# mokemokechicken/reversi-alpha-zero

Measured on AMD Instinct MI355X. Metric: MCTS simulations/sec (self-play, NN included), higher is better.
Workload: dtype f64 tree statistics + f32 net (f16x3 split-operand MFMA trunk)

## Files before the change

### reversi-alpha-zero_amd/csrc/raz_leaf_cache.hip

```cpp
#include <hip/hip_runtime.h>
#include <string.h>
#include "raz_engine.h"
#include "raz_internal.h"

namespace {

constexpr uint32_t kProbes = 8;
enum : uint32_t { ROLE_NONE = 0, ROLE_PLAIN = 1, ROLE_OWN = 2, ROLE_FOLLOW = 3, ROLE_WAIT = 4 };

__device__ __forceinline__ unsigned long long leaf_tag(unsigned long long a, unsigned long long b) {
    unsigned long long x = a * 0x9E3779B97F4A7C15ULL ^ (b + 0xD6E8FEB86659FD93ULL) * 0xC2B2AE3D27D4EB4FULL;
    x ^= x >> 32; x *= 0xFF51AFD7ED558CCDULL; x ^= x >> 29; x *= 0xC4CEB9FE1A85EC53ULL; x ^= x >> 32;
    return x | 1ULL;
}

__global__ __launch_bounds__(256) void k_leaf_claim(raz_leaf_cache_dev C, const unsigned long long* __restrict__ own,
                                                    const unsigned long long* __restrict__ enemy, const uint8_t* __restrict__ active,
                                                    uint32_t p0, uint32_t pn, uint32_t part, uint32_t step) {
    const uint32_t j = blockIdx.x * 256 + threadIdx.x;
    if (j == 0) C.n_compact[part] = 0;
    if (j >= pn) return;
    const uint32_t r = p0 + j;
    if (!active[r]) {
        C.role[r] = ROLE_NONE;
        return;
    }
    const unsigned long long o = own[r], e = enemy[r], tag = leaf_tag(o, e);
    if ((uint32_t)__popcll(o | e) > C.max_discs) {
        C.role[r] = ROLE_PLAIN;
        return;
    }
    const uint32_t h = (uint32_t)(tag >> 24) & C.mask;
    uint32_t role = ROLE_PLAIN;
    for (uint32_t k = 0; k < kProbes; ++k) {
        const uint32_t i = (h + k) & C.mask;
        unsigned long long t = __hip_atomic_load(&C.tags[i], __ATOMIC_RELAXED, __HIP_MEMORY_SCOPE_AGENT);
        if (t == 0) {
            t = atomicCAS(&C.tags[i], 0ULL, tag);
            if (t == 0) {
                C.keys[2 * (size_t)i] = o;
                C.keys[2 * (size_t)i + 1] = e;
                C.stamp[i] = step;
                C.owner[i] = r;
                role = (i << 3) | ROLE_OWN;
                break;
            }
        }
        if (t == tag) {
            role = (i << 3) | ROLE_FOLLOW;
            break;
        }
    }
    if (role == ROLE_PLAIN) atomicAdd(&C.counters[3], 1ULL);
    C.role[r] = role;
}

__global__ __launch_bounds__(256) void k_leaf_resolve(raz_leaf_cache_dev C, const unsigned long long* __restrict__ own,
                                                      const unsigned long long* __restrict__ enemy, uint8_t* __restrict__ active,
                                                      float* __restrict__ policy, float* __restrict__ value, uint32_t p0, uint32_t pn,
                                                      uint32_t part, uint32_t step) {
    const uint32_t j = blockIdx.x * 4 + (threadIdx.x >> 6), lane = threadIdx.x & 63;
    if (j >= pn) return;
    const uint32_t r = p0 + j;
    uint32_t role = __builtin_amdgcn_readfirstlane(C.role[r]);
    const uint32_t kind = role & 7u, i = role >> 3;
    if (kind == ROLE_NONE) return;
    if (kind == ROLE_FOLLOW) {
        const bool same = C.keys[2 * (size_t)i] == own[r] && C.keys[2 * (size_t)i + 1] == enemy[r];
        const uint32_t ow = C.owner[i];
        if (same && __hip_atomic_load(&C.ready[i], __ATOMIC_ACQUIRE, __HIP_MEMORY_SCOPE_AGENT)) {
            policy[(size_t)r * 64 + lane] = C.pv[(size_t)i * 72 + lane];
            if (lane == 0) {
                value[r] = C.pv[(size_t)i * 72 + 64];
                active[r] = 0;
                C.role[r] = ROLE_NONE;
                atomicAdd(&C.counters[0], 1ULL);
            }
            return;
        }
        if (same && C.stamp[i] == step && ow >= p0 && ow < p0 + pn && ow != r) {
            if (lane == 0) {
                active[r] = 0;
                C.role[r] = (i << 3) | ROLE_WAIT;
                atomicAdd(&C.counters[1], 1ULL);
            }
            return;
        }
        role = ROLE_PLAIN;
        if (lane == 0) C.role[r] = ROLE_PLAIN;
    }
    if (lane == 0) {
        const uint32_t ci = atomicAdd(&C.n_compact[part], 1u);
        C.list[p0 + ci] = j;
        atomicAdd(&C.counters[2], 1ULL);
    }
}

__global__ __launch_bounds__(256) void k_leaf_fill(raz_leaf_cache_dev C, float* __restrict__ policy, float* __restrict__ value,
                                                   uint32_t p0, uint32_t pn, uint32_t step) {
    const uint32_t j = blockIdx.x * 4 + (threadIdx.x >> 6), lane = threadIdx.x & 63;
    if (j >= pn) return;
    const uint32_t r = p0 + j, role = C.role[r], kind = role & 7u, i = role >> 3;
    if (kind == ROLE_OWN) {
        if (C.stamp[i] != step || C.owner[i] != r) return;
        C.pv[(size_t)i * 72 + lane] = policy[(size_t)r * 64 + lane];
        if (lane == 0) {
            C.pv[(size_t)i * 72 + 64] = value[r];
            __hip_atomic_store(&C.ready[i], 1u, __ATOMIC_RELEASE, __HIP_MEMORY_SCOPE_AGENT);
        }
    } else if (kind == ROLE_WAIT) {
        const uint32_t ow = C.owner[i];
        policy[(size_t)r * 64 + lane] = policy[(size_t)ow * 64 + lane];
        if (lane == 0) value[r] = value[ow];
    }
}

}

size_t raz_leaf_cache_layout(uint32_t log2_entries, size_t rows, unsigned char* base, raz_leaf_cache_dev* out) {
    const size_t E = (size_t)1 << log2_entries;
    size_t off = 0;
    auto take = [&](size_t bytes) -> unsigned char* {
        unsigned char* p = base ? base + off : nullptr;
        off = (off + bytes + 255) / 256 * 256;
        return p;
    };
    raz_leaf_cache_dev c;
    memset(&c, 0, sizeof c);
    c.tags = (unsigned long long*)take(E * 8);
    c.keys = (unsigned long long*)take(E * 16);
    c.stamp = (uint32_t*)take(E * 4);
    c.owner = (uint32_t*)take(E * 4);
    c.ready = (uint32_t*)take(E * 4);
    c.pv = (float*)take(E * 72 * 4);
    c.counters = (unsigned long long*)take(8 * 8);
    c.n_compact = (uint32_t*)take(16 * 4);
    c.list = (uint32_t*)take(rows * 4);
    c.role = (uint32_t*)take(rows * 4);
    c.mask = (uint32_t)(E - 1);
    c.entries = (uint32_t)E;
    if (out) *out = c;
    return off;
}

int raz_leaf_cache_clear(const raz_leaf_cache_dev& c, size_t rows, hipStream_t s) {
    const size_t E = (size_t)c.entries;
    RAZ_HIP_TRY(hipMemsetAsync(c.tags, 0, E * 8, s), "leaf cache: clear tags");
    RAZ_HIP_TRY(hipMemsetAsync(c.ready, 0, E * 4, s), "leaf cache: clear ready flags");
    RAZ_HIP_TRY(hipMemsetAsync(c.stamp, 0, E * 4, s), "leaf cache: clear stamps");
    RAZ_HIP_TRY(hipMemsetAsync(c.counters, 0, 64, s), "leaf cache: clear counters");
    RAZ_HIP_TRY(hipMemsetAsync(c.n_compact, 0, 64, s), "leaf cache: clear counts");
    RAZ_HIP_TRY(hipMemsetAsync(c.role, 0, rows * 4, s), "leaf cache: clear roles");
    return RAZ_OK;
}

int raz_leaf_cache_before(const raz_leaf_cache_dev& c, const raz_engine_dev& d, uint32_t p0, uint32_t pn, uint32_t part, uint32_t step,
                          hipStream_t s) {
    hipLaunchKernelGGL(k_leaf_claim, dim3((pn + 255) / 256), dim3(256), 0, s, c, d.nn_own, d.nn_enemy, d.nn_active, p0, pn, part, step);
    hipLaunchKernelGGL(k_leaf_resolve, dim3((pn + 3) / 4), dim3(256), 0, s, c, d.nn_own, d.nn_enemy, d.nn_active, d.nn_policy, d.nn_value,
                       p0, pn, part, step);
    return raz_check_launch("raz_engine_step: leaf cache lookup");
}

int raz_leaf_cache_after(const raz_leaf_cache_dev& c, const raz_engine_dev& d, uint32_t p0, uint32_t pn, uint32_t step, hipStream_t s) {
    hipLaunchKernelGGL(k_leaf_fill, dim3((pn + 3) / 4), dim3(256), 0, s, c, d.nn_policy, d.nn_value, p0, pn, step);
    return raz_check_launch("raz_engine_step: leaf cache fill");
}

extern "C" int raz_leaf_cache_probe(int phase, void* d_cache, size_t bytes, uint32_t log2_entries, uint32_t max_discs, size_t rows,
                                    const uint64_t* d_own, const uint64_t* d_enemy, uint8_t* d_active, float* d_policy, float* d_value,
                                    uint32_t p0, uint32_t pn, uint32_t part, uint32_t step, raz_stream_t stream) {
    if (phase < 0 || phase > 2) return raz_fail(RAZ_EINVAL, "raz_leaf_cache_probe: unknown phase");
    if (log2_entries < 10 || log2_entries > 28) return raz_fail(RAZ_EINVAL, "raz_leaf_cache_probe: log2_entries must be 10..28");
    if (!d_cache || ((uintptr_t)d_cache & 255)) return raz_fail(RAZ_EINVAL, "raz_leaf_cache_probe: cache buffer NULL or not 256-byte aligned");
    if (bytes < raz_leaf_cache_layout(log2_entries, rows, nullptr, nullptr)) return raz_fail(RAZ_EINVAL, "raz_leaf_cache_probe: buffer too small (raz_leaf_cache_bytes)");
    if (!d_own || !d_enemy || !d_active || !d_policy || !d_value) return raz_fail(RAZ_EINVAL, "raz_leaf_cache_probe: NULL row buffer");
    if (((uintptr_t)d_own & 7) || ((uintptr_t)d_enemy & 7) || ((uintptr_t)d_policy & 3) || ((uintptr_t)d_value & 3))
        return raz_fail(RAZ_EINVAL, "raz_leaf_cache_probe: misaligned row buffer");
    if ((size_t)p0 + pn > rows) return raz_fail(RAZ_EINVAL, "raz_leaf_cache_probe: slice beyond the rows");
    if (part >= 16) return raz_fail(RAZ_EINVAL, "raz_leaf_cache_probe: part must be below 16");
    if (phase != 0 && pn == 0) return raz_fail(RAZ_EINVAL, "raz_leaf_cache_probe: empty slice");
    raz_leaf_cache_dev c;
    raz_leaf_cache_layout(log2_entries, rows, (unsigned char*)d_cache, &c);
    c.max_discs = max_discs ? max_discs : 64u;
    if (phase == 0) return raz_leaf_cache_clear(c, rows, (hipStream_t)stream);
    raz_engine_dev d;
    memset(&d, 0, sizeof d);
    d.nn_own = (unsigned long long*)d_own;
    d.nn_enemy = (unsigned long long*)d_enemy;
    d.nn_active = d_active;
    d.nn_policy = d_policy;
    d.nn_value = d_value;
    if (phase == 1) return raz_leaf_cache_before(c, d, p0, pn, part, step, (hipStream_t)stream);
    return raz_leaf_cache_after(c, d, p0, pn, step, (hipStream_t)stream);
}
```

### reversi-alpha-zero_amd/csrc/raz_net_f16x3.hip

```cpp
#include <hip/hip_runtime.h>
#include <math.h>
#include <stdlib.h>
#include <string.h>
#include <vector>
#include "raz_bitboard.h"
#include "raz_detmath.h"
#include "raz_internal.h"
#include "raz_net_layout.h"

namespace {

typedef _Float16 h8 __attribute__((ext_vector_type(8)));
typedef _Float16 h4 __attribute__((ext_vector_type(4)));
typedef float f32x4 __attribute__((ext_vector_type(4)));
typedef float f32x16 __attribute__((ext_vector_type(16)));

constexpr int OCT = 128;
constexpr int NWAVE = 8;
constexpr int W_STAGE = 3 * 2 * 2 * OCT * 16;
constexpr int ACT_POS = 4 * 64 * 16;
constexpr int ACT_IMG = NWAVE * ACT_POS + 1280;
constexpr int LDS_W = 0;
constexpr int LDS_ACT = 2 * W_STAGE;
constexpr int LDS_BYTES = LDS_ACT + 2 * ACT_IMG;
constexpr int Z_OFF = NWAVE * ACT_POS;

#ifdef RAZ_F16X3_STAMPS
#define RAZ_STAMP_PARAM , unsigned long long* __restrict__ stamps
#define RAZ_STAMP_ARG , (unsigned long long*)nullptr
#define RAZ_STAMP_BEGIN                                                                                           \
    unsigned long long st_t[8];                                                                                   \
    st_t[0] = __builtin_amdgcn_s_memtime();                                                                       \
    st_t[7] = __builtin_amdgcn_s_memrealtime();                                                                   \
    st_t[6] = (unsigned long long)__builtin_amdgcn_s_getreg((4 << 0) | (0 << 6) | (31 << 11)) | ((unsigned long long)__builtin_amdgcn_s_getreg((20 << 0) | (0 << 6) | (31 << 11)) << 32); \
    st_t[5] = 0;                                                                                                  \
    st_t[1] = st_t[2] = st_t[3] = st_t[4] = 0;                                                                    \
    unsigned long long st_b = 0
#define RAZ_STAMP_BARRIER_IN st_b = __builtin_amdgcn_s_memtime()
#define RAZ_STAMP_BARRIER_OUT(st_)                                    \
    do {                                                              \
        const unsigned long long t_ = __builtin_amdgcn_s_memtime();   \
        st_t[5] += t_ - st_b;                                         \
        if ((st_) == 0) st_t[1] = t_;                                 \
    } while (0)
#define RAZ_STAMP_AT(i_) st_t[i_] = __builtin_amdgcn_s_memtime()
#define RAZ_STAMP_END                                                                                    \
    do {                                                                                                 \
        st_t[3] = __builtin_amdgcn_s_memtime();                                                          \
        __builtin_amdgcn_s_waitcnt(0x0070);                                                \
        st_t[4] = __builtin_amdgcn_s_memtime();                                                          \
        if (lane == 0 && stamps)                                                                         \
            for (int i_ = 0; i_ < 8; ++i_) stamps[((size_t)blockIdx.x * NWAVE + wv) * 8 + i_] = st_t[i_]; \
    } while (0)
#else
#define RAZ_STAMP_PARAM
#define RAZ_STAMP_ARG
#define RAZ_STAMP_BEGIN
#define RAZ_STAMP_BARRIER_IN
#define RAZ_STAMP_BARRIER_OUT(st_)
#define RAZ_STAMP_AT(i_)
#define RAZ_STAMP_END
#endif

#define GLDS16(gptr, lptr)                                                                                      \
    __builtin_amdgcn_global_load_lds((const __attribute__((address_space(1))) void*)(gptr),                     \
                                     (__attribute__((address_space(3))) void*)(lptr), 16, 0, 0)

template <bool SPLIT>
__global__ __launch_bounds__(512, 2) void k_conv3x3_f16x3(const unsigned char* __restrict__ Wl, const float* __restrict__ bias,
                                                          const float* __restrict__ inv_scale_ptr, const unsigned char* in, unsigned char* out,
                                                          const unsigned char* skip, const uint8_t* __restrict__ active, int n, int F,
                                                          unsigned* __restrict__ flag, const uint32_t* __restrict__ n_ptr RAZ_STAMP_PARAM) {
    extern __shared__ __attribute__((aligned(16))) unsigned char lds[];
    const int tid = threadIdx.x, lane = tid & 63, wv = tid >> 6;
    RAZ_STAMP_BEGIN;
    if (n_ptr) n = (int)*n_ptr < n ? (int)*n_ptr : n;
    const int noct = F / OCT, nchunks = F / 16;
    const int b = blockIdx.x;
    const int ot = (b >> 3) % noct;
    const int pg = (b / (8 * noct)) * 8 + (b & 7);
    const int p0 = pg * NWAVE, pos = p0 + wv;
    if (p0 >= n) return;
    const bool live = pos < n && (!active || active[pos]);
    const size_t pos_bytes = (size_t)F * 256;
    const unsigned char* in_pos = in + (size_t)(pos < n ? pos : n - 1) * pos_bytes;
    if (tid < 160) {
        const int im = tid / 80, k = tid % 80;
        ((f32x4*)(lds + LDS_ACT + im * ACT_IMG + Z_OFF))[k] = (f32x4){0.f, 0.f, 0.f, 0.f};
    }
    const int kg = lane >> 5;
    uint32_t boff[2][9];
#pragma unroll
    for (int nt = 0; nt < 2; ++nt) {
        const int sq = nt * 32 + (lane & 31), y = sq >> 3, x = sq & 7;
#pragma unroll
        for (int t = 0; t < 9; ++t) {
            const int yy = y + t / 3 - 1, xx = x + t % 3 - 1;
            const bool ok = yy >= 0 && yy < 8 && xx >= 0 && xx < 8;
            const int s2 = sq + (t / 3 - 1) * 8 + (t % 3 - 1);
            boff[nt][t] = ok ? (uint32_t)(wv * ACT_POS + kg * 2048 + s2 * 16) : (uint32_t)(Z_OFF + (s2 & 15) * 16);
        }
    }
    const uint32_t aoff = (uint32_t)(kg * 4096 + (lane & 31) * 16);
    f32x16 acc[4][2];
#pragma unroll
    for (int m = 0; m < 4; ++m)
#pragma unroll
        for (int nt = 0; nt < 2; ++nt)
#pragma unroll
            for (int r = 0; r < 16; ++r) acc[m][nt][r] = 0.f;
    const unsigned char* wsrc = Wl + (size_t)ot * nchunks * 3 * W_STAGE + lane * 16;
    const unsigned char* asrc = in_pos + lane * 16;
    auto issue = [&](int c, int tg) {
        const int st = c * 3 + tg;
        const unsigned char* src = wsrc + (size_t)st * W_STAGE;
        unsigned char* dst = lds + LDS_W + (st & 1) * W_STAGE;
        if constexpr (SPLIT) {
#pragma unroll
            for (int i = 0; i < 3; ++i) GLDS16(src + (wv * 3 + i) * 1024, dst + (wv * 3 + i) * 1024);
        } else {
            const int p0w = (wv >> 1) * 4 + (wv & 1);
            GLDS16(src + p0w * 1024, dst + p0w * 1024);
            if (wv < 4) GLDS16(src + (p0w + 16) * 1024, dst + (p0w + 16) * 1024);
        }
        if (tg == 0) {
            const unsigned char* a = asrc + (size_t)c * ACT_POS;
            unsigned char* ad = lds + LDS_ACT + (c & 1) * ACT_IMG + wv * ACT_POS;
#pragma unroll
            for (int pl = 0; pl < 4; pl += SPLIT ? 1 : 2) GLDS16(a + pl * 1024, ad + pl * 1024);
        }
    };
    issue(0, 0);
    for (int c = 0; c < nchunks; ++c) {
        const uint32_t abase = (uint32_t)(LDS_ACT + (c & 1) * ACT_IMG);
#pragma unroll
        for (int tg = 0; tg < 3; ++tg) {
            const int st = c * 3 + tg;
            RAZ_STAMP_BARRIER_IN;
            __syncthreads();
            RAZ_STAMP_BARRIER_OUT(st);
            if (tg < 2) issue(c, tg + 1);
            else if (c + 1 < nchunks) issue(c + 1, 0);
            const uint32_t wbase = (uint32_t)(LDS_W + (st & 1) * W_STAGE) + aoff;
#pragma unroll
            for (int tt = 0; tt < 3; ++tt) {
                const int t = tg * 3 + tt;
                if constexpr (SPLIT) {
                    h8 bh[2], bl[2];
#pragma unroll
                    for (int nt = 0; nt < 2; ++nt) {
                        bh[nt] = *(const h8*)(lds + abase + boff[nt][t]);
                        bl[nt] = *(const h8*)(lds + abase + boff[nt][t] + 1024);
                    }
#pragma unroll
                    for (int m = 0; m < 4; ++m) {
                        const h8 ah = *(const h8*)(lds + wbase + tt * 8192 + m * 512);
                        const h8 al = *(const h8*)(lds + wbase + tt * 8192 + m * 512 + 2048);
#pragma unroll
                        for (int nt = 0; nt < 2; ++nt) {
                            acc[m][nt] = __builtin_amdgcn_mfma_f32_32x32x16_f16(al, bh[nt], acc[m][nt], 0, 0, 0);
                            acc[m][nt] = __builtin_amdgcn_mfma_f32_32x32x16_f16(ah, bl[nt], acc[m][nt], 0, 0, 0);
                            acc[m][nt] = __builtin_amdgcn_mfma_f32_32x32x16_f16(ah, bh[nt], acc[m][nt], 0, 0, 0);
                        }
                    }
                } else {
                    h8 bh[2];
#pragma unroll
                    for (int nt = 0; nt < 2; ++nt) bh[nt] = *(const h8*)(lds + abase + boff[nt][t]);
#pragma unroll
                    for (int m = 0; m < 4; ++m) {
                        const h8 ah = *(const h8*)(lds + wbase + tt * 8192 + m * 512);
#pragma unroll
                        for (int nt = 0; nt < 2; ++nt) acc[m][nt] = __builtin_amdgcn_mfma_f32_32x32x16_f16(ah, bh[nt], acc[m][nt], 0, 0, 0);
                    }
                }
            }
        }
    }
    RAZ_STAMP_AT(2);
    if (!live) return;
    const float inv_scale = *inv_scale_ptr;
    unsigned char* out_pos = out + (size_t)pos * pos_bytes;
    const unsigned char* skip_pos = skip ? skip + (size_t)pos * pos_bytes : nullptr;
    bool over = false;
#pragma unroll
    for (int m = 0; m < 4; ++m)
#pragma unroll
        for (int q = 0; q < 4; ++q) {
            const int oc8 = ot * OCT + m * 32 + q * 8;
            const f32x4 bv = *(const f32x4*)(bias + oc8 + 4 * kg);
            const size_t unit = (size_t)(oc8 >> 4) * ACT_POS + (size_t)((oc8 >> 3) & 1) * 2048;
#pragma unroll
            for (int nt = 0; nt < 2; ++nt) {
                const size_t o = unit + (size_t)(nt * 32 + (lane & 31)) * 16 + kg * 8;
                float v[4];
#pragma unroll
                for (int j = 0; j < 4; ++j) v[j] = acc[m][nt][q * 4 + j] * inv_scale + bv[j];
                if (skip_pos) {
                    if constexpr (SPLIT) {
                        const h4 sh = *(const h4*)(skip_pos + o), sl = *(const h4*)(skip_pos + o + 1024);
#pragma unroll
                        for (int j = 0; j < 4; ++j) v[j] = v[j] + ((float)sh[j] + (float)sl[j]);
                    } else {
                        const h4 sh = *(const h4*)(skip_pos + o);
#pragma unroll
                        for (int j = 0; j < 4; ++j) v[j] = v[j] + (float)sh[j];
                    }
                }
                h4 hi, lo;
#pragma unroll
                for (int j = 0; j < 4; ++j) {
                    const float r = v[j] > 0.0f ? v[j] : 0.0f;
                    over |= !(r < 60000.0f);
                    hi[j] = (_Float16)r;
                    lo[j] = (_Float16)(r - (float)hi[j]);
                }
                *(h4*)(out_pos + o) = hi;
                if constexpr (SPLIT) *(h4*)(out_pos + o + 1024) = lo;
            }
        }
    if (over) flag[(size_t)pos * RAZ_NET_ROWFLAG_WORDS] = 1u;
    RAZ_STAMP_END;
}

template <bool SPLIT>
__global__ __launch_bounds__(256) void k_conv0_split(const float* __restrict__ W0, const raz_bb* __restrict__ own,
                                                     const raz_bb* __restrict__ enemy, const uint8_t* __restrict__ active,
                                                     unsigned char* out, int n, int F, unsigned* __restrict__ flag,
                                                     const uint32_t* __restrict__ list, const uint32_t* __restrict__ n_ptr) {
    const int pos = blockIdx.x, lane = threadIdx.x & 63;
    const int wv = __builtin_amdgcn_readfirstlane(threadIdx.x >> 6);
    if (threadIdx.x == 0) {
        flag[(size_t)pos * RAZ_NET_ROWFLAG_WORDS] = 0u;
        if (pos == 0) flag[1] = 0u;
    }
    __syncthreads();
    if (n_ptr) n = (int)*n_ptr < n ? (int)*n_ptr : n;
    if (pos >= n || (!list && active && !active[pos])) return;
    bool over = false;
    const size_t src = list ? list[pos] : (size_t)pos;
    const raz_bb bo = own[src], be = enemy[src];
    const int y = lane >> 3, x = lane & 7;
    float x0[9], x1[9];
#pragma unroll
    for (int t = 0; t < 9; ++t) {
        const int yy = y + t / 3 - 1, xx = x + t % 3 - 1;
        const bool ok = (yy >= 0) && (yy < 8) && (xx >= 0) && (xx < 8);
        const int s = (yy * 8 + xx) & 63;
        x0[t] = ok ? (float)((bo >> s) & 1) : 0.0f;
        x1[t] = ok ? (float)((be >> s) & 1) : 0.0f;
    }
    const float* bias = W0 + (size_t)F * 18;
    unsigned char* op = out + (size_t)pos * F * 256;
    for (int ocb = wv; ocb < F / 16; ocb += 4) {
        float acc[16];
#pragma unroll
        for (int o = 0; o < 16; ++o) acc[o] = bias[ocb * 16 + o];
#pragma unroll
        for (int t = 0; t < 9; ++t) {
            const float* wt = W0 + ((size_t)ocb * 9 + t) * 32;
#pragma unroll
            for (int o = 0; o < 16; ++o) acc[o] = fmaf(x0[t], wt[o], acc[o]);
#pragma unroll
            for (int o = 0; o < 16; ++o) acc[o] = fmaf(x1[t], wt[16 + o], acc[o]);
        }
#pragma unroll
        for (int g = 0; g < 2; ++g) {
            h8 hi, lo;
#pragma unroll
            for (int j = 0; j < 8; ++j) {
                const float r = acc[g * 8 + j] > 0.0f ? acc[g * 8 + j] : 0.0f;
                over |= !(r < 60000.0f);
                hi[j] = (_Float16)r;
                lo[j] = (_Float16)(r - (float)hi[j]);
            }
            *(h8*)(op + (size_t)ocb * ACT_POS + (g * 2 + 0) * 1024 + lane * 16) = hi;
            if constexpr (SPLIT) *(h8*)(op + (size_t)ocb * ACT_POS + (g * 2 + 1) * 1024 + lane * 16) = lo;
        }
    }
    if (over) flag[(size_t)pos * RAZ_NET_ROWFLAG_WORDS] = 1u;
}

template <bool SPLIT>
__global__ __launch_bounds__(64) void k_heads_split(const float* __restrict__ H, const unsigned char* trunk,
                                                    const uint8_t* __restrict__ active, float* __restrict__ policy,
                                                    float* __restrict__ value, int n, int F, int V,
                                                    const uint32_t* __restrict__ list, const uint32_t* __restrict__ n_ptr) {
    extern __shared__ __attribute__((aligned(16))) float head[];
    const int pos = blockIdx.x, lane = threadIdx.x;
    if (n_ptr) n = (int)*n_ptr < n ? (int)*n_ptr : n;
    if (pos >= n || (!list && active && !active[pos])) return;
    const size_t dst = list ? list[pos] : (size_t)pos;
    const float* pol_w = H;
    const float* pol_b = pol_w + 2 * F;
    const float* pfc_w = pol_b + 2;
    const float* pfc_b = pfc_w + 128 * 64;
    const float* val_w = pfc_b + 64;
    const float* val_b = val_w + F;
    const float* v1_w = val_b + 1;
    const float* v1_b = v1_w + 64 * V;
    const float* v2_w = v1_b + V;
    const float* v2_b = v2_w + V;
    float* ph = head;
    float* vh = head + 128;
    float* h1 = head + 192;
    const unsigned char* a = trunk + (size_t)pos * F * 256 + lane * 16;
    float p0 = pol_b[0], p1 = pol_b[1], v0 = val_b[0];
    for (int c = 0; c < F / 16; ++c) {
#pragma unroll
        for (int g = 0; g < 2; ++g) {
            const h8 hi = *(const h8*)(a + (size_t)c * ACT_POS + (g * 2 + 0) * 1024);
            h8 lo = hi;
            if constexpr (SPLIT) lo = *(const h8*)(a + (size_t)c * ACT_POS + (g * 2 + 1) * 1024);
#pragma unroll
            for (int j = 0; j < 8; ++j) {
                const int ic = c * 16 + g * 8 + j;
                const float xv = SPLIT ? (float)hi[j] + (float)lo[j] : (float)hi[j];
                p0 = fmaf(xv, pol_w[ic], p0);
                p1 = fmaf(xv, pol_w[F + ic], p1);
                v0 = fmaf(xv, val_w[ic], v0);
            }
        }
    }
    ph[lane] = p0 > 0.0f ? p0 : 0.0f;
    ph[64 + lane] = p1 > 0.0f ? p1 : 0.0f;
    vh[lane] = v0 > 0.0f ? v0 : 0.0f;
    __syncthreads();
    float logit = pfc_b[lane];
#pragma unroll 16
    for (int j = 0; j < 128; ++j) logit = fmaf(ph[j], pfc_w[j * 64 + lane], logit);
    float m = logit;
#pragma unroll
    for (int s = 1; s < 64; s <<= 1) m = fmaxf(m, __shfl_xor(m, s));
    const float e = raz_det_expf(logit - m);
    float sum = e;
#pragma unroll
    for (int s = 1; s < 64; s <<= 1) sum = sum + __shfl_xor(sum, s);
    policy[dst * 64 + lane] = e / sum;
    for (int o0 = 0; o0 < V; o0 += 64) {
        const int o = o0 + lane;
        if (o < V) {
            float acc = v1_b[o];
#pragma unroll 8
            for (int j = 0; j < 64; ++j) acc = fmaf(vh[j], v1_w[j * V + o], acc);
            h1[o] = acc > 0.0f ? acc : 0.0f;
        }
    }
    __syncthreads();
    float acc = v2_b[0];
    for (int j = 0; j < V; ++j) acc = fmaf(h1[j], v2_w[j], acc);
    if (lane == 0) value[dst] = raz_det_tanhf(acc);
}

}

void raz_net_build_f16x3(const float* src, float* dst, int F, int R, int V) {
    const float* lsrc = src + ((size_t)F * 18 + F);
    float* scales = dst + f16x3_scale_off(F, R, V);
    const int nchunks = F / 16, noct = F / 128;
    for (int l = 1; l < 2 * R + 1; ++l) {
        float mx = 0.f;
        for (size_t i = 0; i < (size_t)F * F * 9; ++i) mx = fmaxf(mx, fabsf(lsrc[i]));
        int e = 0;
        if (mx > 0.f) frexpf(mx, &e);
        const float S = ldexpf(1.0f, 15 - e);
        scales[l - 1] = ldexpf(1.0f, e - 15);
        _Float16* w = (_Float16*)(dst + f16x3_layer_off(F, R, V, l));
        for (int ot = 0; ot < noct; ++ot)
            for (int c = 0; c < nchunks; ++c)
                for (int t = 0; t < 9; ++t)
                    for (int kg = 0; kg < 2; ++kg)
                        for (int o = 0; o < 128; ++o)
                            for (int j = 0; j < 8; ++j) {
                                const int oc = ot * 128 + o, ic = c * 16 + kg * 8 + j;
                                const float v = lsrc[((size_t)oc * F + ic) * 9 + t] * S;
                                const _Float16 hi = (_Float16)v, lo = (_Float16)(v - (float)hi);
                                const size_t stage = ((size_t)ot * nchunks + c) * 3 + t / 3;
                                const size_t base = stage * (W_STAGE / 2) + ((size_t)(t % 3) * 2 + kg) * 2 * 128 * 8;
                                w[base + (size_t)o * 8 + j] = hi;
                                w[base + 128 * 8 + (size_t)o * 8 + j] = lo;
                            }
        lsrc += (size_t)F * F * 9 + F;
    }
}

static int heads_launch(bool split, const float* W, int F, int R, int V, const unsigned char* trunk, const uint8_t* active, float* policy,
                        float* value, size_t n, hipStream_t s, const uint32_t* list, const uint32_t* n_ptr) {
    const auto heads = split ? k_heads_split<true> : k_heads_split<false>;
    hipLaunchKernelGGL(heads, dim3((unsigned)n), dim3(64), (192 + (size_t)V) * sizeof(float), s,
                       W + heads_off(F, R), trunk, active, policy, value, (int)n, F, V, list, n_ptr);
    return raz_check_launch("raz_net_forward (split heads)");
}
int raz_net_heads_split(const float* W, int F, int R, int V, const unsigned char* trunk, const uint8_t* active, float* policy, float* value,
                        size_t n, hipStream_t s, const uint32_t* list, const uint32_t* n_ptr) {
    return heads_launch(true, W, F, R, V, trunk, active, policy, value, n, s, list, n_ptr);
}

size_t raz_net_f16x3_scratch_bytes(int F, size_t n) { return n * ((size_t)2 * F * 256 + RAZ_NET_ROWFLAG_WORDS * 4); }

__global__ __launch_bounds__(256) void k_flag_unrepaired(const unsigned* __restrict__ rowflag, unsigned* __restrict__ sticky, int n,
                                                         const uint32_t* __restrict__ n_ptr) {
    const int i = blockIdx.x * 256 + threadIdx.x;
    const int rows = n_ptr ? ((int)*n_ptr < n ? (int)*n_ptr : n) : n;
    if (i < rows && rowflag[(size_t)i * RAZ_NET_ROWFLAG_WORDS]) atomicOr(sticky, 1u);
}
static int raz_net_flag_unrepaired(const unsigned* rowflag, unsigned* sticky, size_t n, const uint32_t* n_ptr, hipStream_t s) {
    hipLaunchKernelGGL(k_flag_unrepaired, dim3((unsigned)((n + 255) / 256)), dim3(256), 0, s, rowflag, sticky, (int)n, n_ptr);
    return raz_check_launch("raz_net_forward (range flags)");
}

unsigned* raz_net_f16x3_flag(const float* W, int F, int R, int V) { return (unsigned*)(W + f16x3_scale_off(F, R, V) + (size_t)2 * R + 8); }

int raz_net_forward_f16x3(const float* W, int F, int R, int V, const uint64_t* own, const uint64_t* enemy,
                          const uint8_t* active, float* policy, float* value, size_t n, void* scratch, size_t scratch_bytes,
                          hipStream_t s, const uint32_t* list, const uint32_t* n_ptr, bool split) {
    if (!scratch || scratch_bytes < raz_net_f16x3_scratch_bytes(F, n))
        return raz_fail(RAZ_ENOMEM, "raz_net_forward: scratch too small (raz_net_scratch_bytes)");
    unsigned char* bufA = (unsigned char*)scratch;
    unsigned char* bufT = bufA + (size_t)n * F * 256;
    unsigned* sticky = raz_net_f16x3_flag(W, F, R, V);
    unsigned* flag = (unsigned*)(bufT + (size_t)n * F * 256);
    const float* scales = W + f16x3_scale_off(F, R, V);
    const auto conv = split ? k_conv3x3_f16x3<true> : k_conv3x3_f16x3<false>;
    {
        static unsigned long long attr_devices[2] = {0, 0};
        int dev = 0;
        RAZ_HIP_TRY(hipGetDevice(&dev), "raz_net_forward: hipGetDevice");
        if (dev >= 64 || !(attr_devices[split] >> dev & 1)) {
            RAZ_HIP_TRY(hipFuncSetAttribute((const void*)conv, hipFuncAttributeMaxDynamicSharedMemorySize, LDS_BYTES), "raz_net_forward: hipFuncSetAttribute");
            if (dev < 64) attr_devices[split] |= 1ull << dev;
        }
    }
    const unsigned conv_threads = NWAVE * 64;
    const auto conv0 = split ? k_conv0_split<true> : k_conv0_split<false>;
    hipLaunchKernelGGL(conv0, dim3((unsigned)n), dim3(256), 0, s, W + conv_off(F, 0), (const raz_bb*)own,
                       (const raz_bb*)enemy, active, bufA, (int)n, F, flag, list, n_ptr);
    const unsigned groups = (unsigned)((n + NWAVE - 1) / NWAVE);
    const unsigned tiles = ((groups + 7) / 8) * 8 * (unsigned)(F / 128);
    const unsigned grid = tiles;
    for (int r = 0; r < R; ++r) {
        const int l1 = 1 + 2 * r, l2 = 2 + 2 * r;
        hipLaunchKernelGGL(conv, dim3(grid), dim3(conv_threads), LDS_BYTES, s,
                           (const unsigned char*)(W + f16x3_layer_off(F, R, V, l1)), W + conv_off(F, l1) + (size_t)F * 9 * F,
                           scales + (l1 - 1), (const unsigned char*)bufA, bufT, (const unsigned char*)nullptr, list ? nullptr : active, (int)n, F, flag, n_ptr RAZ_STAMP_ARG);
        hipLaunchKernelGGL(conv, dim3(grid), dim3(conv_threads), LDS_BYTES, s,
                           (const unsigned char*)(W + f16x3_layer_off(F, R, V, l2)), W + conv_off(F, l2) + (size_t)F * 9 * F,
                           scales + (l2 - 1), (const unsigned char*)bufT, bufA, (const unsigned char*)bufA, list ? nullptr : active, (int)n, F, flag, n_ptr RAZ_STAMP_ARG);
    }
    const int rc = heads_launch(split, W, F, R, V, bufA, active, policy, value, n, s, list, n_ptr);
    if (rc != RAZ_OK) return rc;
    if (!f16x3_repairs(F, V))
        return raz_net_flag_unrepaired(flag, sticky, n, n_ptr, s);
    return raz_net_repair_rows(W, F, R, V, own, enemy, policy, value, n, flag, sticky, list, n_ptr, s);
}
```

Measured before the change: 354,100.

## Aggregate leaf-resolve atomics per block, widen conv epilogue stores, batch conv0 rows

```diff
diff --git a/reversi-alpha-zero_amd/csrc/raz_leaf_cache.hip b/reversi-alpha-zero_amd/csrc/raz_leaf_cache.hip
--- a/reversi-alpha-zero_amd/csrc/raz_leaf_cache.hip
+++ b/reversi-alpha-zero_amd/csrc/raz_leaf_cache.hip
@@ -55,44 +55,79 @@
     C.role[r] = role;
 }
 
+constexpr uint32_t kResolveRows = 256;
+enum : uint32_t { FATE_NONE = 0, FATE_NET = 1, FATE_HIT = 2, FATE_WAIT = 3 };
+
 __global__ __launch_bounds__(256) void k_leaf_resolve(raz_leaf_cache_dev C, const unsigned long long* __restrict__ own,
                                                       const unsigned long long* __restrict__ enemy, uint8_t* __restrict__ active,
                                                       float* __restrict__ policy, float* __restrict__ value, uint32_t p0, uint32_t pn,
                                                       uint32_t part, uint32_t step) {
-    const uint32_t j = blockIdx.x * 4 + (threadIdx.x >> 6), lane = threadIdx.x & 63;
-    if (j >= pn) return;
-    const uint32_t r = p0 + j;
-    uint32_t role = __builtin_amdgcn_readfirstlane(C.role[r]);
-    const uint32_t kind = role & 7u, i = role >> 3;
-    if (kind == ROLE_NONE) return;
-    if (kind == ROLE_FOLLOW) {
-        const bool same = C.keys[2 * (size_t)i] == own[r] && C.keys[2 * (size_t)i + 1] == enemy[r];
-        const uint32_t ow = C.owner[i];
-        if (same && __hip_atomic_load(&C.ready[i], __ATOMIC_ACQUIRE, __HIP_MEMORY_SCOPE_AGENT)) {
-            policy[(size_t)r * 64 + lane] = C.pv[(size_t)i * 72 + lane];
-            if (lane == 0) {
-                value[r] = C.pv[(size_t)i * 72 + 64];
+    __shared__ uint32_t s_count[4][3];
+    __shared__ uint32_t s_base;
+    __shared__ uint32_t s_hit_row[kResolveRows];
+    __shared__ uint32_t s_hit_entry[kResolveRows];
+    const uint32_t tid = threadIdx.x, lane = tid & 63, wv = tid >> 6;
+    const uint32_t j0 = blockIdx.x * kResolveRows, j = j0 + tid;
+    uint32_t fate = FATE_NONE, i = 0;
+    if (j < pn) {
+        const uint32_t r = p0 + j, role = C.role[r], kind = role & 7u;
+        i = role >> 3;
+        if (kind == ROLE_FOLLOW) {
+            const bool same = C.keys[2 * (size_t)i] == own[r] && C.keys[2 * (size_t)i + 1] == enemy[r];
+            const uint32_t ow = C.owner[i];
+            if (same && __hip_atomic_load(&C.ready[i], __ATOMIC_ACQUIRE, __HIP_MEMORY_SCOPE_AGENT)) {
+                fate = FATE_HIT;
                 active[r] = 0;
                 C.role[r] = ROLE_NONE;
-                atomicAdd(&C.counters[0], 1ULL);
-            }
-            return;
-        }
-        if (same && C.stamp[i] == step && ow >= p0 && ow < p0 + pn && ow != r) {
-            if (lane == 0) {
+            } else if (same && C.stamp[i] == step && ow >= p0 && ow < p0 + pn && ow != r) {
+                fate = FATE_WAIT;
                 active[r] = 0;
                 C.role[r] = (i << 3) | ROLE_WAIT;
-                atomicAdd(&C.counters[1], 1ULL);
+            } else {
+                fate = FATE_NET;
+                C.role[r] = ROLE_PLAIN;
             }
-            return;
-        }
-        role = ROLE_PLAIN;
-        if (lane == 0) C.role[r] = ROLE_PLAIN;
-    }
+        } else if (kind != ROLE_NONE) {
+            fate = FATE_NET;
+        }
+    }
+    const unsigned long long m_net = __ballot(fate == FATE_NET), m_hit = __ballot(fate == FATE_HIT), m_wait = __ballot(fate == FATE_WAIT);
     if (lane == 0) {
-        const uint32_t ci = atomicAdd(&C.n_compact[part], 1u);
-        C.list[p0 + ci] = j;
-        atomicAdd(&C.counters[2], 1ULL);
+        s_count[wv][0] = (uint32_t)__popcll(m_net);
+        s_count[wv][1] = (uint32_t)__popcll(m_hit);
+        s_count[wv][2] = (uint32_t)__popcll(m_wait);
+    }
+    __syncthreads();
+    uint32_t net_before = 0, hit_before = 0, n_net = 0, n_hit = 0, n_wait = 0;
+#pragma unroll
+    for (uint32_t w = 0; w < 4; ++w) {
+        if (w < wv) {
+            net_before += s_count[w][0];
+            hit_before += s_count[w][1];
+        }
+        n_net += s_count[w][0];
+        n_hit += s_count[w][1];
+        n_wait += s_count[w][2];
+    }
+    if (tid == 0) {
+        s_base = n_net ? atomicAdd(&C.n_compact[part], n_net) : 0u;
+        if (n_hit) atomicAdd(&C.counters[0], (unsigned long long)n_hit);
+        if (n_wait) atomicAdd(&C.counters[1], (unsigned long long)n_wait);
+        if (n_net) atomicAdd(&C.counters[2], (unsigned long long)n_net);
+    }
+    const unsigned long long below = (1ULL << lane) - 1ULL;
+    if (fate == FATE_HIT) {
+        const uint32_t h = hit_before + (uint32_t)__popcll(m_hit & below);
+        s_hit_row[h] = tid;
+        s_hit_entry[h] = i;
+    }
+    __syncthreads();
+    if (fate == FATE_NET)
+        C.list[p0 + s_base + net_before + (uint32_t)__popcll(m_net & below)] = j;
+    for (uint32_t h = wv; h < n_hit; h += 4) {
+        const size_t r = (size_t)p0 + j0 + s_hit_row[h], e = s_hit_entry[h];
+        policy[r * 64 + lane] = C.pv[e * 72 + lane];
+        if (lane == 0) value[r] = C.pv[e * 72 + 64];
     }
 }
 
@@ -157,7 +192,7 @@
 int raz_leaf_cache_before(const raz_leaf_cache_dev& c, const raz_engine_dev& d, uint32_t p0, uint32_t pn, uint32_t part, uint32_t step,
                           hipStream_t s) {
     hipLaunchKernelGGL(k_leaf_claim, dim3((pn + 255) / 256), dim3(256), 0, s, c, d.nn_own, d.nn_enemy, d.nn_active, p0, pn, part, step);
-    hipLaunchKernelGGL(k_leaf_resolve, dim3((pn + 3) / 4), dim3(256), 0, s, c, d.nn_own, d.nn_enemy, d.nn_active, d.nn_policy, d.nn_value,
+    hipLaunchKernelGGL(k_leaf_resolve, dim3((pn + kResolveRows - 1) / kResolveRows), dim3(256), 0, s, c, d.nn_own, d.nn_enemy, d.nn_active, d.nn_policy, d.nn_value,
                        p0, pn, part, step);
     return raz_check_launch("raz_engine_step: leaf cache lookup");
 }
diff --git a/reversi-alpha-zero_amd/csrc/raz_net_f16x3.hip b/reversi-alpha-zero_amd/csrc/raz_net_f16x3.hip
--- a/reversi-alpha-zero_amd/csrc/raz_net_f16x3.hip
+++ b/reversi-alpha-zero_amd/csrc/raz_net_f16x3.hip
@@ -62,6 +62,19 @@
 #define RAZ_STAMP_END
 #endif
 
+__device__ __forceinline__ void halves_trade(float a, float b, int upper, float& first, float& second) {
+#ifdef RAZ_WAVE_EMU
+    const float got = __shfl_xor(upper ? a : b, 32);
+    first = upper ? got : a;
+    second = upper ? b : got;
+#else
+    (void)upper;
+    const auto r = __builtin_amdgcn_permlane32_swap(__float_as_uint(a), __float_as_uint(b), false, false);
+    first = __uint_as_float(r[0]);
+    second = __uint_as_float(r[1]);
+#endif
+}
+
 #define GLDS16(gptr, lptr)                                                                                      \
     __builtin_amdgcn_global_load_lds((const __attribute__((address_space(1))) void*)(gptr),                     \
                                      (__attribute__((address_space(3))) void*)(lptr), 16, 0, 0)
@@ -180,105 +193,151 @@
     RAZ_STAMP_AT(2);
     if (!live) return;
     const float inv_scale = *inv_scale_ptr;
-    unsigned char* out_pos = out + (size_t)pos * pos_bytes;
-    const unsigned char* skip_pos = skip ? skip + (size_t)pos * pos_bytes : nullptr;
-    bool over = false;
-#pragma unroll
-    for (int m = 0; m < 4; ++m)
+    unsigned char* out_pos = out + (size_t)pos * pos_bytes + lane * 16;
+    const unsigned char* skip_pos = skip ? skip + (size_t)pos * pos_bytes + lane * 16 : nullptr;
+    h8 skh[2][4], skl[2][4];
+    auto load_skip = [&](int m) {
 #pragma unroll
         for (int q = 0; q < 4; ++q) {
             const int oc8 = ot * OCT + m * 32 + q * 8;
-            const f32x4 bv = *(const f32x4*)(bias + oc8 + 4 * kg);
             const size_t unit = (size_t)(oc8 >> 4) * ACT_POS + (size_t)((oc8 >> 3) & 1) * 2048;
-#pragma unroll
-            for (int nt = 0; nt < 2; ++nt) {
-                const size_t o = unit + (size_t)(nt * 32 + (lane & 31)) * 16 + kg * 8;
-                float v[4];
-#pragma unroll
-                for (int j = 0; j < 4; ++j) v[j] = acc[m][nt][q * 4 + j] * inv_scale + bv[j];
-                if (skip_pos) {
-                    if constexpr (SPLIT) {
-                        const h4 sh = *(const h4*)(skip_pos + o), sl = *(const h4*)(skip_pos + o + 1024);
-#pragma unroll
-                        for (int j = 0; j < 4; ++j) v[j] = v[j] + ((float)sh[j] + (float)sl[j]);
-                    } else {
-                        const h4 sh = *(const h4*)(skip_pos + o);
-#pragma unroll
-                        for (int j = 0; j < 4; ++j) v[j] = v[j] + (float)sh[j];
-                    }
+            skh[m & 1][q] = *(const h8*)(skip_pos + unit);
+            if constexpr (SPLIT) skl[m & 1][q] = *(const h8*)(skip_pos + unit + 1024);
+        }
+    };
+    if (skip_pos) load_skip(0);
+    bool over = false;
+#pragma unroll
+    for (int m = 0; m < 4; ++m) {
+        if (skip_pos && m + 1 < 4) load_skip(m + 1);
+#pragma unroll
+        for (int q = 0; q < 4; ++q) {
+            const int oc8 = ot * OCT + m * 32 + q * 8;
+            const size_t unit = (size_t)(oc8 >> 4) * ACT_POS + (size_t)((oc8 >> 3) & 1) * 2048;
+            float v[8];
+#pragma unroll
+            for (int j = 0; j < 4; ++j) halves_trade(acc[m][0][q * 4 + j], acc[m][1][q * 4 + j], kg, v[j], v[4 + j]);
+#pragma unroll
+            for (int j = 0; j < 8; ++j) v[j] = v[j] * inv_scale + bias[oc8 + j];
+            if (skip_pos) {
+                const h8 sh = skh[m & 1][q];
+                if constexpr (SPLIT) {
+                    const h8 sl = skl[m & 1][q];
+#pragma unroll
+                    for (int j = 0; j < 8; ++j) v[j] = v[j] + ((float)sh[j] + (float)sl[j]);
+                } else {
+#pragma unroll
+                    for (int j = 0; j < 8; ++j) v[j] = v[j] + (float)sh[j];
                 }
-                h4 hi, lo;
-#pragma unroll
-                for (int j = 0; j < 4; ++j) {
-                    const float r = v[j] > 0.0f ? v[j] : 0.0f;
+            }
+            h8 hi, lo;
+#pragma unroll
+            for (int j = 0; j < 8; ++j) {
+                const float r = v[j] > 0.0f ? v[j] : 0.0f;
+                over |= !(r < 60000.0f);
+                hi[j] = (_Float16)r;
+                lo[j] = (_Float16)(r - (float)hi[j]);
+            }
+            *(h8*)(out_pos + unit) = hi;
+            if constexpr (SPLIT) *(h8*)(out_pos + unit + 1024) = lo;
+        }
+    }
+    if (over) flag[(size_t)pos * RAZ_NET_ROWFLAG_WORDS] = 1u;
+    RAZ_STAMP_END;
+}
+
+typedef float f32x2 __attribute__((ext_vector_type(2)));
+constexpr int CONV0_ROWS = 2;
+
+template <bool SPLIT>
+__global__ __launch_bounds__(256, 6) void k_conv0_split(const float* __restrict__ W0, const raz_bb* __restrict__ own,
+                                                        const raz_bb* __restrict__ enemy, const uint8_t* __restrict__ active,
+                                                        unsigned char* out, int n, int F, unsigned* __restrict__ flag,
+                                                        const uint32_t* __restrict__ list, const uint32_t* __restrict__ n_ptr) {
+    const int posA = blockIdx.x * CONV0_ROWS, posB = posA + 1, lane = threadIdx.x & 63;
+    const int wv = __builtin_amdgcn_readfirstlane(threadIdx.x >> 6);
+    if (threadIdx.x == 0) {
+        flag[(size_t)posA * RAZ_NET_ROWFLAG_WORDS] = 0u;
+        if (posB < n) flag[(size_t)posB * RAZ_NET_ROWFLAG_WORDS] = 0u;
+        if (posA == 0) flag[1] = 0u;
+    }
+    __syncthreads();
+    if (n_ptr) n = (int)*n_ptr < n ? (int)*n_ptr : n;
+    const bool liveA = posA < n && (list || !active || active[posA]);
+    const bool liveB = posB < n && (list || !active || active[posB]);
+    if (!liveA && !liveB) return;
+    raz_bb bo[2] = {0, 0}, be[2] = {0, 0};
+    if (liveA) {
+        const size_t src = list ? list[posA] : (size_t)posA;
+        bo[0] = own[src];
+        be[0] = enemy[src];
+    }
+    if (liveB) {
+        const size_t src = list ? list[posB] : (size_t)posB;
+        bo[1] = own[src];
+        be[1] = enemy[src];
+    }
+    const int y = lane >> 3, x = lane & 7;
+    f32x2 x0[9], x1[9];
+#pragma unroll
+    for (int t = 0; t < 9; ++t) {
+        const int yy = y + t / 3 - 1, xx = x + t % 3 - 1;
+        const bool ok = (yy >= 0) && (yy < 8) && (xx >= 0) && (xx < 8);
+        const int s = (yy * 8 + xx) & 63;
+#pragma unroll
+        for (int k = 0; k < 2; ++k) {
+            x0[t][k] = ok ? (float)(uint32_t)((bo[k] >> s) & 1) : 0.0f;
+            x1[t][k] = ok ? (float)(uint32_t)((be[k] >> s) & 1) : 0.0f;
+        }
+    }
+    const float* bias = W0 + (size_t)F * 18;
+    unsigned char* op = out + (size_t)posA * F * 256 + lane * 16;
+    bool overA = false, overB = false;
+    for (int ocb = wv; ocb < F / 16; ocb += 4) {
+#pragma unroll 1
+        for (int g = 0; g < 2; ++g) {
+            f32x2 acc[8];
+#pragma unroll
+            for (int o = 0; o < 8; ++o) {
+                const float b = bias[ocb * 16 + g * 8 + o];
+                acc[o] = (f32x2){b, b};
+            }
+#pragma unroll
+            for (int t = 0; t < 9; ++t) {
+                const float* wt = W0 + ((size_t)ocb * 9 + t) * 32 + g * 8;
+#pragma unroll
+                for (int o = 0; o < 8; ++o) {
+                    const float w = wt[o];
+                    acc[o] = __builtin_elementwise_fma(x0[t], (f32x2){w, w}, acc[o]);
+                }
+#pragma unroll
+                for (int o = 0; o < 8; ++o) {
+                    const float w = wt[16 + o];
+                    acc[o] = __builtin_elementwise_fma(x1[t], (f32x2){w, w}, acc[o]);
+                }
+            }
+#pragma unroll
+            for (int k = 0; k < 2; ++k) {
+                if (!(k ? liveB : liveA)) continue;
+                h8 hi, lo;
+                bool over = false;
+#pragma unroll
+                for (int j = 0; j < 8; ++j) {
+                    const float r = acc[j][k] > 0.0f ? acc[j][k] : 0.0f;
                     over |= !(r < 60000.0f);
                     hi[j] = (_Float16)r;
                     lo[j] = (_Float16)(r - (float)hi[j]);
                 }
-                *(h4*)(out_pos + o) = hi;
-                if constexpr (SPLIT) *(h4*)(out_pos + o + 1024) = lo;
-            }
-        }
-    if (over) flag[(size_t)pos * RAZ_NET_ROWFLAG_WORDS] = 1u;
-    RAZ_STAMP_END;
-}
-
-template <bool SPLIT>
-__global__ __launch_bounds__(256) void k_conv0_split(const float* __restrict__ W0, const raz_bb* __restrict__ own,
-                                                     const raz_bb* __restrict__ enemy, const uint8_t* __restrict__ active,
-                                                     unsigned char* out, int n, int F, unsigned* __restrict__ flag,
-                                                     const uint32_t* __restrict__ list, const uint32_t* __restrict__ n_ptr) {
-    const int pos = blockIdx.x, lane = threadIdx.x & 63;
-    const int wv = __builtin_amdgcn_readfirstlane(threadIdx.x >> 6);
-    if (threadIdx.x == 0) {
-        flag[(size_t)pos * RAZ_NET_ROWFLAG_WORDS] = 0u;
-        if (pos == 0) flag[1] = 0u;
-    }
-    __syncthreads();
-    if (n_ptr) n = (int)*n_ptr < n ? (int)*n_ptr : n;
-    if (pos >= n || (!list && active && !active[pos])) return;
-    bool over = false;
-    const size_t src = list ? list[pos] : (size_t)pos;
-    const raz_bb bo = own[src], be = enemy[src];
-    const int y = lane >> 3, x = lane & 7;
-    float x0[9], x1[9];
-#pragma unroll
-    for (int t = 0; t < 9; ++t) {
-        const int yy = y + t / 3 - 1, xx = x + t % 3 - 1;
-        const bool ok = (yy >= 0) && (yy < 8) && (xx >= 0) && (xx < 8);
-        const int s = (yy * 8 + xx) & 63;
-        x0[t] = ok ? (float)((bo >> s) & 1) : 0.0f;
-        x1[t] = ok ? (float)((be >> s) & 1) : 0.0f;
-    }
-    const float* bias = W0 + (size_t)F * 18;
-    unsigned char* op = out + (size_t)pos * F * 256;
-    for (int ocb = wv; ocb < F / 16; ocb += 4) {
-        float acc[16];
-#pragma unroll
-        for (int o = 0; o < 16; ++o) acc[o] = bias[ocb * 16 + o];
-#pragma unroll
-        for (int t = 0; t < 9; ++t) {
-            const float* wt = W0 + ((size_t)ocb * 9 + t) * 32;
-#pragma unroll
-            for (int o = 0; o < 16; ++o) acc[o] = fmaf(x0[t], wt[o], acc[o]);
-#pragma unroll
-            for (int o = 0; o < 16; ++o) acc[o] = fmaf(x1[t], wt[16 + o], acc[o]);
-        }
-#pragma unroll
-        for (int g = 0; g < 2; ++g) {
-            h8 hi, lo;
-#pragma unroll
-            for (int j = 0; j < 8; ++j) {
-                const float r = acc[g * 8 + j] > 0.0f ? acc[g * 8 + j] : 0.0f;
-                over |= !(r < 60000.0f);
-                hi[j] = (_Float16)r;
-                lo[j] = (_Float16)(r - (float)hi[j]);
-            }
-            *(h8*)(op + (size_t)ocb * ACT_POS + (g * 2 + 0) * 1024 + lane * 16) = hi;
-            if constexpr (SPLIT) *(h8*)(op + (size_t)ocb * ACT_POS + (g * 2 + 1) * 1024 + lane * 16) = lo;
-        }
-    }
-    if (over) flag[(size_t)pos * RAZ_NET_ROWFLAG_WORDS] = 1u;
+                if (k) overB |= over;
+                else overA |= over;
+                unsigned char* o16 = op + (size_t)k * F * 256 + (size_t)ocb * ACT_POS + (g * 2) * 1024;
+                *(h8*)o16 = hi;
+                if constexpr (SPLIT) *(h8*)(o16 + 1024) = lo;
+            }
+        }
+    }
+    if (overA) flag[(size_t)posA * RAZ_NET_ROWFLAG_WORDS] = 1u;
+    if (overB) flag[(size_t)posB * RAZ_NET_ROWFLAG_WORDS] = 1u;
 }
 
 template <bool SPLIT>
@@ -433,7 +492,7 @@
     }
     const unsigned conv_threads = NWAVE * 64;
     const auto conv0 = split ? k_conv0_split<true> : k_conv0_split<false>;
-    hipLaunchKernelGGL(conv0, dim3((unsigned)n), dim3(256), 0, s, W + conv_off(F, 0), (const raz_bb*)own,
+    hipLaunchKernelGGL(conv0, dim3((unsigned)((n + CONV0_ROWS - 1) / CONV0_ROWS)), dim3(256), 0, s, W + conv_off(F, 0), (const raz_bb*)own,
                        (const raz_bb*)enemy, active, bufA, (int)n, F, flag, list, n_ptr);
     const unsigned groups = (unsigned)((n + NWAVE - 1) / NWAVE);
     const unsigned tiles = ((groups + 7) / 8) * 8 * (unsigned)(F / 128);
```

Measured after the change: 375,800, median of 6. 6.1% higher.
